# avabag01-ai/spectrogram-midi

Measured on AMD Instinct MI355X. Metric: audio-seconds transcribed/sec (44.1 kHz, n_fft=2048), higher is better.
Workload: dtype f64

## Files before the change

spectrogram-midi_amd/csrc/kernels.hip:

```cpp
#include "kernels.h"
#include "fft8.h"
#include "rake_decide.h"

#include <algorithm>
#include <cfloat>
#include <cmath>
#include <cstdlib>
#include <cstring>
#include <type_traits>

namespace aegis {

__device__ __forceinline__ int find_clip(const int64_t *__restrict__ frame_off, int n_clips, int64_t f) {
    int lo = 0, hi = n_clips;
    while (hi - lo > 1) {
        const int mid = (lo + hi) >> 1;
        if (frame_off[mid] <= f) lo = mid; else hi = mid;
    }
    return lo;
}

__device__ __forceinline__ int64_t geo_n_sel(const PassParams &p) { return p.ctl ? p.ctl->n_sel : p.n_sel; }
__device__ __forceinline__ int64_t geo_t_begin(const PassParams &p) { return p.ctl ? p.ctl->t_begin : p.t_begin; }
__device__ __forceinline__ int64_t geo_vt_begin(const PassParams &p) { return p.ctl ? p.ctl->vt_begin : p.vt_begin; }
// ... 343 lines not shown
                    v[q] = make_double2((double)xs[i], i < 1024 ? (double)xs[1024 - i] : 0.0);
                }
                fft8_pass1_write(z, tid, v);
                __syncthreads();
                if (want_rms && tid < 16) {
                    const float *r = red + tid * 8;
                    blk[tid] = ((r[0] + r[1]) + (r[2] + r[3])) + ((r[4] + r[5]) + (r[6] + r[7]));
                }
                fft8_read8(z, tid, v);
                __syncthreads();
                fft8_pass_write<8>(z, tid, v, twr.p2);
                __syncthreads();
                fft8_read8(z, tid, v);
                __syncthreads();
                fft8_pass_write<64>(z, tid, v, twr.p3);
                __syncthreads();
                fft8_pass4(z, tid, twr);
                __syncthreads();
            }
            FRM_TICK(2)
            if (want_rms && tid == 0 && live) {
                float b0 = (blk[0] + blk[1]) + (blk[2] + blk[3]);
                float b1 = (blk[4] + blk[5]) + (blk[6] + blk[7]);
                float b2 = (blk[8] + blk[9]) + (blk[10] + blk[11]);
                float b3 = (blk[12] + blk[13]) + (blk[14] + blk[15]);
                const float total = 0.0f + ((b0 + b1) + (b2 + b3));
                p.out_rms[fo] = sqrtf(total / 2048.0f);
            }
            if (!want_fft) continue;

            if (tid < 205) {
                auto zpair = [&](int k, double2 &zk, double2 &zn) { zk = z[zsw(k & 2047)]; zn = z[zsw((2048 - k) & 2047)]; };
                auto Afrom = [](const double2 &zk, const double2 &zn) { return make_double2(zk.x + zn.x, zk.y - zn.y); };
                const int k0 = 5 * tid;
                double2 zk, zn, zk1, zn1;
                zpair(k0 - 1, zk, zn);
                double2 Am = Afrom(zk, zn);
                zpair(k0, zk, zn);
                double2 A = Afrom(zk, zn);
#pragma unroll
                for (int r = 0; r < 5; ++r) {
                    const int k = k0 + r;
                    zpair(k + 1, zk1, zn1);
                    const double2 Ap = Afrom(zk1, zn1);
                    if (want_pyin) {
                        const double2 Bv = make_double2(zk.y + zn.y, zn.x - zk.x);
                        P[h][r] = c_mul(A, Bv);
                    }
                    if (want_mel) {
                        const float re = (float)(0.125 * (2.0 * A.x - (Am.x + Ap.x)));
                        const float im = (float)(0.125 * (2.0 * A.y - (Am.y + Ap.y)));
                        const float mag = (float)sqrt((double)re * (double)re + (double)im * (double)im);
                        (h == 0 ? pw : pw1)[k] = mag * mag;
                    }
                    Am = A; A = Ap; zk = zk1; zn = zn1;
                }
            }
            if (want_mel && h == 1 && tid < 15) pw1[1025 + tid] = 0.0f;
            __syncthreads();
            FRM_TICK(3)
        }
        __builtin_amdgcn_s_waitcnt(kWaitVmcnt0);
        if (want_mel) {
            if (has_chunk) {
                const float4 *wp = reinterpret_cast<const float4 *>(tb.mel_chunk_w) + tid * 4;
                const float4 w0 = wp[0], w1 = wp[1], w2 = wp[2], w3 = wp[3];
#pragma unroll
                for (int h = 0; h < 2; ++h) {
                    const float *pp = (h == 0 ? pw : pw1) + mel_bin;
                    float acc = 0.0f;
                    acc = fmaf(w0.x, pp[0], acc); acc = fmaf(w0.y, pp[1], acc); acc = fmaf(w0.z, pp[2], acc); acc = fmaf(w0.w, pp[3], acc);
                    acc = fmaf(w1.x, pp[4], acc); acc = fmaf(w1.y, pp[5], acc); acc = fmaf(w1.z, pp[6], acc); acc = fmaf(w1.w, pp[7], acc);
                    acc = fmaf(w2.x, pp[8], acc); acc = fmaf(w2.y, pp[9], acc); acc = fmaf(w2.z, pp[10], acc); acc = fmaf(w2.w, pp[11], acc);
                    acc = fmaf(w3.x, pp[12], acc); acc = fmaf(w3.y, pp[13], acc); acc = fmaf(w3.z, pp[14], acc); acc = fmaf(w3.w, pp[15], acc);
                    (h == 0 ? part : part1)[tid] = acc;
                }
            }
            __syncthreads();
            {
                const int h = wid >> 1, bt = tid & 127;
                const bool live = flive[h];
                const float *pt = h == 0 ? part : part1;
                float acc = 0.0f;
                if (bt < p.n_mels && live) {
                    const int c0 = band_c0, c1 = band_c1;
                    float pv[6];
#pragma unroll
                    for (int k = 0; k < 6; ++k) pv[k] = pt[min(c0 + k, 255)];
                    acc = c0 < c1 ? pv[0] : 0.0f;
#pragma unroll
                    for (int k = 1; k < 6; ++k) if (c0 + k < c1) acc = acc + pv[k];
                    for (int cidx = c0 + 6; cidx < c1; ++cidx) acc = acc + pt[cidx];
                    p.melpow[fidx[h] * p.n_mels + bt] = acc;
                }
                const unsigned m = wave_umax(__float_as_uint(acc));
                if (lane == 0 && live) atomicMax(&p.clipmax[fclip[h]], m);
            }
            if (!want_pyin) __syncthreads();
        }
        FRM_TICK(4)
        if (!want_pyin) continue;

        if (tid < 205) {
#pragma unroll
            for (int r = 0; r < 5; ++r) {
                const int k = 5 * tid + r;
                const double2 u = P[0][r], v = P[1][r];
                z[zsw(k)] = make_double2(u.x - v.y, -u.y - v.x);
                if (k > 0 && k < 1024) z[zsw(2048 - k)] = make_double2(u.x + v.y, u.y - v.x);
            }
        }
        __syncthreads();
        {
            double2 v[8];
            fft8_read8(z, tid, v);
            __syncthreads();
            fft8_pass1_write(z, tid, v);
            __syncthreads();
            fft8_read8(z, tid, v);
            __syncthreads();
            fft8_pass_write<8>(z, tid, v, twr.p2);
            __syncthreads();
            fft8_read8(z, tid, v);
            __syncthreads();
            fft8_pass_write<64>(z, tid, v, twr.p3);
            __syncthreads();
            fft8_pass4_lags(z, tid, twr, mp);
            __syncthreads();
        }
        FRM_TICK(5)
        const bool keep_first = p.cmnd_in_frame != 0;
        if (keep_first) {
            float es[2][3];
#pragma unroll
            for (int h = 0; h < 2; ++h) {
                const float *row = en + (pr + h) * en_stride;
                float en0 = row[0];
                if (fabsf(en0) < 1e-6f) en0 = 0.0f;
#pragma unroll
                for (int u = 0; u < 3; ++u) {
                    float e = row[min(tid + 256 * u, mp)];
                    if (fabsf(e) < 1e-6f) e = 0.0f;
                    es[h][u] = en0 + e;
                }
            }
            __syncthreads();
            double *__restrict__ d0 = reinterpret_cast<double *>(en + pr * en_stride);
            double *__restrict__ d1 = p.dfn + fidx[1] * (int64_t)p.lag_stride;
#pragma unroll
            for (int u = 0; u < 3; ++u) {
                const int tau = tid + 256 * u;
                if (tau <= mp) {
                    const double2 zz = z[zsw(1024 + tau)];
                    double a0 = zz.x * (1.0 / 8192.0), a1 = -zz.y * (1.0 / 8192.0);
                    if (fabs(a0) < 1e-6) a0 = 0.0;
                    if (fabs(a1) < 1e-6) a1 = 0.0;
                    if constexpr (INJECT) {
                        if (flive[0]) d0[tau] = inj[fout[0] * (int64_t)(mp + 1) + tau];
                        if (flive[1]) d1[tau] = inj[fout[1] * (int64_t)(mp + 1) + tau];
                    } else {
                        if (flive[0]) d0[tau] = (double)es[0][u] - 2.0 * a0;
                        if (flive[1]) d1[tau] = (double)es[1][u] - 2.0 * a1;
                    }
                }
            }
        } else {
#pragma unroll
        for (int h = 0; h < 2; ++h) {
            if (!flive[h]) continue;
            const float *row = en + (pr + h) * en_stride;
            float en0 = row[0];
            if (fabsf(en0) < 1e-6f) en0 = 0.0f;
            double *__restrict__ drow = p.dfn + fidx[h] * (int64_t)p.lag_stride;
            for (int tau = tid; tau <= mp; tau += 256) {
                const double2 zz = z[zsw(1024 + tau)];
                double a = (h == 0 ? zz.x : -zz.y) * (1.0 / 8192.0);
                if (fabs(a) < 1e-6) a = 0.0;
                float e = row[tau];
                if (fabsf(e) < 1e-6f) e = 0.0f;
                const float esum = en0 + e;
                if constexpr (INJECT) drow[tau] = inj[fout[h] * (int64_t)(mp + 1) + tau];
                else drow[tau] = (double)esum - 2.0 * a;
            }
        }
        }
        FRM_TICK(6)
    }
    if (want_pyin && p.cmnd_in_frame) {
        const int RS = frame_cmnd_stride(mp), minp = p.min_period;
        double *zrows = reinterpret_cast<double *>(fsm);
        auto row_of = [&](int i) { return (i & 1) ? zrows + (i >> 1) * RS : reinterpret_cast<double *>(en + i * en_stride); };
        __syncthreads();
        double dv[kFramesPerWg][3];
        int64_t fr[kFramesPerWg];
#pragma unroll
        for (int i = 0; i < kFramesPerWg; ++i) fr[i] = i < nfr ? frow[i] : -1;
#pragma unroll
        for (int i = 0; i < kFramesPerWg; ++i) {
            const double *__restrict__ src = (i & 1) ? p.dfn + (fr[i] < 0 ? 0 : fr[i]) * (int64_t)p.lag_stride : row_of(i);
#pragma unroll
            for (int u = 0; u < 3; ++u) {
                const int tau = tid + 256 * u;
                dv[i][u] = (fr[i] >= 0 && tau <= mp) ? src[tau] : 0.0;
            }
        }
#pragma unroll
        for (int i = 1; i < kFramesPerWg; i += 2) {
#pragma unroll
            for (int u = 0; u < 3; ++u) {
                const int tau = tid + 256 * u;
                if (i < nfr && tau <= mp) zrows[(i >> 1) * RS + tau] = dv[i][u];
            }
        }
        __syncthreads();
        FRM_TICK(7)
        if (wid == 0) __builtin_amdgcn_s_setprio(3);
        if (wid == 0 && lane < nfr) cmnd_walk(row_of(lane), mp);
        if (wid == 0) __builtin_amdgcn_s_setprio(0);
        __syncthreads();
        FRM_TICK(8)
        const bool troughs = p.troughs != 0;
#pragma unroll
        for (int i = 0; i < kFramesPerWg; ++i) {
            double *__restrict__ drow = p.dfn + (fr[i] < 0 ? 0 : fr[i]) * (int64_t)p.lag_stride;
            double *__restrict__ cs = row_of(i);
#pragma unroll
            for (int u = 0; u < 3; ++u) {
                const int tau = tid + 256 * u;
                if (fr[i] >= 0 && tau >= minp && tau <= mp) {
                    const double yv = dv[i][u] / (cs[tau] / (double)tau + DBL_MIN);
                    if (troughs) cs[tau] = yv;
                    else drow[tau] = yv;
                }
            }
        }
        FRM_TICK(9)
        if (troughs) {
            __syncthreads();
            const int nl = p.n_lags, KM = trough_km(nl), NR = (nl + 63) >> 6;
            const unsigned long long below = (1ull << lane) - 1ull;
            for (int i = wid; i < nfr; i += 4) {
                if (fr[i] < 0) continue;
                const double *__restrict__ y = row_of(i) + minp;
                double *__restrict__ trow = p.dfn + fr[i] * (int64_t)p.lag_stride;
                int16_t *__restrict__ tiv = reinterpret_cast<int16_t *>(trow + 8 + 2 * KM);
                int K = 0;
                for (int r = 0; r < NR; ++r) {
                    const int k = 64 * r + lane;
                    bool tr = false;
                    double ym = 0.0, y0 = 0.0, yp = 0.0;
                    if (k < nl) {
                        y0 = y[k];
                        if (k > 0) ym = y[k - 1];
                        if (k < nl - 1) yp = y[k + 1];
                        if (k == 0) tr = y0 < yp;
                        else if (k == nl - 1) tr = y0 < ym;
                        else tr = (y0 < ym) && (y0 <= yp);
                    }
                    const unsigned long long m = __ballot(tr);
                    if (tr) {
                        const int pos = K + __popcll(m & below);
                        double shift = 0.0;
                        if (k > 0 && k < nl - 1) {
                            const double a = yp + ym - 2.0 * y0;
                            const double b = (yp - ym) / 2.0;
                            if (fabs(b) < fabs(a)) shift = -b / a;
                        }
                        trow[8 + pos] = y0;
                        trow[8 + KM + pos] = shift;
                        tiv[pos] = (int16_t)k;
                    }
                    K += __popcll(m);
                }
                if (lane == 0) trow[0] = __longlong_as_double((long long)K);
            }
        }
    }
#if defined(AEGIS_ABLATE) && (AEGIS_ABLATE & 128)
    if (blockIdx.x == 1000 && (tid == 0 || tid == 64)) { for (int k = 0; k < 10; ++k) g_frm_dbg[(tid ? 12 : 0) + k] = facc[k]; }
#endif
}
#if defined(AEGIS_ABLATE) && (AEGIS_ABLATE & 128)
hipError_t frame_debug_fetch(long long *dst) { return hipMemcpyFromSymbol(dst, HIP_SYMBOL(g_frm_dbg), sizeof(long long) * 24); }
#else
hipError_t frame_debug_fetch(long long *dst) { for (int i = 0; i < 24; ++i) dst[i] = 0; return hipSuccess; }
#endif

constexpr int kKMax = 512;
constexpr int kMaxRounds = 8;

template <int CTRL, int ROW_MASK>
__device__ __forceinline__ int dpp_imin(int v) {
    return min(v, __builtin_amdgcn_update_dpp(v, v, CTRL, ROW_MASK, 0xf, false));
}
__device__ __forceinline__ int wave_min_i32(int v) {
    v = dpp_imin<0x111, 0xf>(v);
    v = dpp_imin<0x112, 0xf>(v);
    v = dpp_imin<0x114, 0xf>(v);
    v = dpp_imin<0x118, 0xf>(v);
    v = dpp_imin<0x142, 0xa>(v);
    v = dpp_imin<0x143, 0xc>(v);
    return __builtin_amdgcn_readlane(v, 63);
}

__device__ __forceinline__ void wave_sync() {
    __builtin_amdgcn_fence(__ATOMIC_SEQ_CST, "wavefront");
    __builtin_amdgcn_wave_barrier();
}

#if defined(AEGIS_ABLATE) && (AEGIS_ABLATE & 256)
__device__ long long g_obs_dbg[16];
#define OBS_TICK(k) { const long long now__ = clock64(); oacc[k] += now__ - olast; olast = now__; }
#else
#define OBS_TICK(k)
#endif
__global__ __launch_bounds__(512, 4) void pyin_obs_kernel(PassParams p, DevTables tb, int frames_per_wave) {
    extern __shared__ __align__(16) unsigned char osm[];
    const int nl = p.n_lags, B = p.n_bins;
    const int KM = nl / 2 + 2;
    const int YN = (max(nl, B) + 1) & ~1;
    const int DN = (p.max_period + 1 + 32 + 1) & ~1;
    const int UN = (max(DN, 2 * KM + (4 * KM + 7) / 8) + 1) & ~1;
    const int TN = (2 * (KM + 1) + 101 + 1) & ~1;
    const int lane = threadIdx.x & 63;
    const int wid = __builtin_amdgcn_readfirstlane((int)(threadIdx.x >> 6)), nwaves = (int)(blockDim.x >> 6);
    double *bfact = reinterpret_cast<double *>(osm);
    double *bexp = bfact + (KM + 1);
    double *bcum = bexp + (KM + 1);
    double *y = bfact + TN + (size_t)wid * (YN + UN);
    double *row = y;
    double *dd = y + YN;
    double *th = dd;
    double *tp = th + KM;
    int16_t *ti = reinterpret_cast<int16_t *>(tp + KM);
    int16_t *tbin = ti + KM;
    __shared__ double beta_s[104];

#if defined(AEGIS_ABLATE) && (AEGIS_ABLATE & 256)
    long long oacc[12] = {0, 0, 0, 0, 0, 0, 0, 0, 0, 0, 0, 0}, olast = clock64();
#endif
    for (int i = threadIdx.x; i < 100; i += blockDim.x) beta_s[i] = tb.beta_probs[i];
    for (int i = threadIdx.x; i <= KM; i += blockDim.x) { bfact[i] = tb.boltz_fact[i]; bexp[i] = tb.boltz_exp[i]; }
    for (int i = threadIdx.x; i <= 100; i += blockDim.x) bcum[i] = tb.beta_cumsum[i];
    __syncthreads();

    int64_t f = 0, fo = 0, sel_end = 0;
    int Kn = -1;
    const int64_t n_sel = geo_n_sel(p);
    for (int it = 0; it < frames_per_wave; ++it) {
    const int64_t fsel = ((int64_t)blockIdx.x * nwaves + wid) * frames_per_wave + it;
    if (fsel >= n_sel) break;
    if (it > 0 && fsel < sel_end) { ++f; ++fo; }
    else {
        int c;
        int64_t t;
        map_frame(p, fsel, c, t, f);
        fo = out_index(p, c, t);
        sel_end = p.sel_off[c + 1];
    }
    const int mp = p.max_period, minp = p.min_period;
    const double *__restrict__ dr = p.dfn + f * (int64_t)p.lag_stride;
    wave_sync();
    int K = 0;
    double *tsh = y;
    if (p.troughs) {
        const int KMt = trough_km(nl);
        if (Kn >= 0) K = Kn;
        else {
        K = __builtin_amdgcn_readfirstlane((int)__double_as_longlong(dr[0]));
        const int16_t *__restrict__ tiv = reinterpret_cast<const int16_t *>(dr + 8 + 2 * KMt);
        for (int k = lane; k < K; k += 64) {
            const double h = dr[8 + k], sh = dr[8 + KMt + k];
            const int16_t ix = tiv[k];
            th[k] = h; tsh[k] = sh; ti[k] = ix;
        }
        }
        wave_sync();
        OBS_TICK(0)
    } else {
    if (p.cmnd_in_frame) {
        for (int base = lane; base < nl; base += 320) {
            double t5[5];
#pragma unroll
            for (int u = 0; u < 5; ++u) t5[u] = dr[minp + min(base + 64 * u, nl - 1)];
#pragma unroll
            for (int u = 0; u < 5; ++u) if (base + 64 * u < nl) y[base + 64 * u] = t5[u];
        }
        wave_sync();
        OBS_TICK(0)
    } else {
    for (int base = lane; base <= mp; base += 320) {
        double t5[5];
#pragma unroll
        for (int u = 0; u < 5; ++u) t5[u] = dr[min(base + 64 * u, mp)];
#pragma unroll
        for (int u = 0; u < 5; ++u) if (base + 64 * u <= mp) dd[base + 64 * u] = t5[u];
    }
    wave_sync();
    OBS_TICK(0)
    if (lane == 0) {
        double cs = dd[1];
        if (minp <= 1) y[1 - minp] = cs;
        int tau = 2;
        constexpr int GL = 8;
        double2 ra[GL / 2], rb[GL / 2];
        auto request = [&](double2 (&r)[GL / 2], int t0) {
#pragma unroll
            for (int i = 0; i < GL / 2; ++i) r[i] = *reinterpret_cast<const double2 *>(dd + t0 + 2 * i);
        };
        auto group = [&](auto all_tag, double2 (&cur)[GL / 2], double2 (&nxt)[GL / 2], int t0) {
            constexpr bool ALL = decltype(all_tag)::value;
            request(nxt, t0 + GL);
            double *yo = y + (t0 - minp);
#pragma unroll
            for (int i = 0; i < GL / 2; ++i) {
                cs = cs + cur[i].x; if (ALL || t0 + 2 * i >= minp) yo[2 * i] = cs;
                cs = cs + cur[i].y; if (ALL || t0 + 2 * i + 1 >= minp) yo[2 * i + 1] = cs;
            }
        };
        request(ra, tau);
        bool in_a = true;
        for (; tau < minp && tau + GL - 1 <= mp; tau += GL, in_a = !in_a) {
            if (in_a) group(std::false_type{}, ra, rb, tau); else group(std::false_type{}, rb, ra, tau);
        }
        if (!in_a && tau + GL - 1 <= mp) { group(std::true_type{}, rb, ra, tau); tau += GL; }
        for (; tau + 2 * GL - 1 <= mp; tau += 2 * GL) { group(std::true_type{}, ra, rb, tau); group(std::true_type{}, rb, ra, tau + GL); }
        if (tau + GL - 1 <= mp) { group(std::true_type{}, ra, rb, tau); tau += GL; }
        for (; tau <= mp; ++tau) { cs = cs + dd[tau]; if (tau >= minp) y[tau - minp] = cs; }
    }
    wave_sync();
    OBS_TICK(1)
    for (int i = lane; i < nl; i += 64) {
        const int tau = i + minp;
        y[i] = dd[tau] / (y[i] / (double)tau + DBL_MIN);
    }
    if (p.yin != nullptr) {
        wave_sync();
        double *__restrict__ yo = p.yin + f * (int64_t)p.yin_stride;
        for (int i = lane; i < nl; i += 64) yo[i] = y[i];
    }
    wave_sync();
    }

    OBS_TICK(2)
    const int CH = (nl + 63) >> 6;
    unsigned mask = 0;
    int cnt = 0;
    for (int r = 0; r < CH; ++r) {
        const int i = lane * CH + r;
        if (i < nl) {
            const double yi = y[i];
            bool tr;
            if (i == 0) tr = yi < y[1];
            else if (i == nl - 1) tr = yi < y[i - 1];
            else tr = (yi < y[i - 1]) && (yi <= y[i + 1]);
            if (tr) { mask |= 1u << r; ++cnt; }
        }
    }
    const int incl = wave_incl_scan(cnt, lane);
    K = __shfl(incl, 63);
    {
        int k = incl - cnt;
        for (int r = 0; r < CH; ++r)
            if (mask & (1u << r)) { const int i = lane * CH + r; th[k] = y[i]; ti[k] = (int16_t)i; ++k; }
    }
    wave_sync();
    }

    OBS_TICK(3)
    double vp = 0.0;
    unsigned segm = 0;
    const int rounds = (K + 63) >> 6;
    const bool ahead = p.troughs && it + 1 < frames_per_wave && fsel + 1 < sel_end;
    double nK = 0.0, nh[2] = {0.0, 0.0}, nsh[2] = {0.0, 0.0};
    int16_t nix[2] = {0, 0};
    auto tail = [&](auto maxr_tag) {
        constexpr int MAXR = decltype(maxr_tag)::value;
        if (K > 0) {
            int jk[MAXR];
            double acc[MAXR];
            int jmin = 101;
    #pragma unroll
            for (int q = 0; q < MAXR; ++q) {
                jk[q] = 101; acc[q] = 0.0;
                if (q < rounds) {
                    const int k = q * 64 + lane;
                    if (k < K) {
                        const double h = th[k];
                        int g;
                        if (!(h < 1.0)) g = 100;
                        else if (h <= 0.0) g = 0;
                        else g = (int)(h * 100.0);
                        auto thr = [](int i) { return i >= 100 ? 1.0 : (double)i * 0.01; };
                        while (g < 100 && !(h < thr(g + 1))) ++g;
                        while (g > 0 && h < thr(g)) --g;
                        jk[q] = g;
                        jmin = min(jmin, g);
                    }
                }
            }
            jmin = wave_min_i32(jmin);
            OBS_TICK(4)

            const unsigned long long lt_mask = (1ull << lane) - 1ull;
            int j = jmin;
            while (j < 100) {
                unsigned long long M[MAXR];
                int nj = 0, nxt = 100;
    #pragma unroll
                for (int q = 0; q < MAXR; ++q) {
                    M[q] = 0ull;
                    if (q < rounds) {
                        M[q] = __ballot(jk[q] <= j);
                        nj += __popcll(M[q]);
                        if (jk[q] > j) nxt = min(nxt, jk[q]);
                    }
                }
                nxt = wave_min_i32(nxt);
                const double fact = bfact[nj];
                double prior[MAXR];
                int before = 0;
    #pragma unroll
                for (int q = 0; q < MAXR; ++q) {
                    prior[q] = 0.0;
                    if (q < rounds) {
                        if (jk[q] <= j) prior[q] = fact * bexp[before + __popcll(M[q] & lt_mask)];
                        before += __popcll(M[q]);
                    }
                }
                for (int jj = j; jj < nxt; ++jj) {
                    const double bj = beta_s[jj];
    #pragma unroll
                    for (int q = 0; q < MAXR; ++q)
                        if (q < rounds) acc[q] = acc[q] + prior[q] * bj;
                }
                j = nxt;
            }

            OBS_TICK(5)
            double bh = INFINITY;
            int bk = kKMax;
    #pragma unroll
            for (int q = 0; q < MAXR; ++q) {
                const int k = q * 64 + lane;
                if (q < rounds && k < K) { const double h = th[k]; if (h < bh) { bh = h; bk = k; } }
            }
    #pragma unroll
            for (int o = 32; o >= 1; o >>= 1) {
                const double oh = __shfl_xor(bh, o);
                const int ok = __shfl_xor(bk, o);
                if (oh < bh || (oh == bh && ok < bk)) { bh = oh; bk = ok; }
            }
    #pragma unroll
            for (int q = 0; q < MAXR; ++q) {
                if (q < rounds && q * 64 + lane == bk) {
                    const int nb = jk[q] > 100 ? 100 : jk[q];
                    acc[q] = acc[q] + 0.01 * bcum[nb];
                }
            }

    #pragma unroll
            for (int q = 0; q < MAXR; ++q) {
                const int k = q * 64 + lane;
                if (q < rounds && k < K) {
                    const double pr = acc[q];
                    int bin = -1;
                    if (pr != 0.0) {
                        const int i = ti[k];
                        double shift = 0.0;
                        if (p.troughs) shift = tsh[k];
                        else if (i > 0 && i < nl - 1) {
                            const double ym = y[i - 1], y0 = y[i], yp = y[i + 1];
                            const double a = yp + ym - 2.0 * y0;
                            const double b = (yp - ym) / 2.0;
                            if (fabs(b) < fabs(a)) shift = -b / a;
                        }
                        const double period = (double)(p.min_period + i) + shift;
                        const double f0c = (double)p.sr / period;
                        double r = rint(120.0 * log2(f0c / p.fmin));
                        r = !(r >= 0.0) ? 0.0 : (r > (double)B ? (double)B : r);
                        bin = (int)r;
                    }
                    tp[k] = pr;
                    tbin[k] = (int16_t)bin;
                }
            }
        }
        OBS_TICK(6)
        if (ahead) {
            const int KMt = trough_km(nl);
            const double *__restrict__ drn = dr + p.lag_stride;
            const int16_t *__restrict__ tivn = reinterpret_cast<const int16_t *>(drn + 8 + 2 * KMt);
            nK = drn[0];
    #pragma unroll
            for (int q = 0; q < 2; ++q) {
                const int k = min(q * 64 + lane, KMt - 1);
                nh[q] = drn[8 + k]; nsh[q] = drn[8 + KMt + k]; nix[q] = tivn[k];
            }
        }
        wave_sync();
        for (int b = lane; b < B; b += 64) row[b] = p.log_tiny;
        wave_sync();
        if (K > 0) {
            bool winq[MAXR];
            double prq[MAXR];
            unsigned lseg = 0;
            int binq[MAXR];
            unsigned long long hasm[MAXR];
    #pragma unroll
            for (int q = 0; q < MAXR; ++q) {
                const int k = q * 64 + lane;
                binq[q] = (q < rounds && k < K) ? (int)tbin[k] : -1;
                hasm[q] = __ballot(binq[q] >= 0);
            }
    #pragma unroll
            for (int q = 0; q < MAXR; ++q) {
                winq[q] = false; prq[q] = 0.0;
                const int bin = binq[q];
                if (bin >= 0 && bin < B) {
                    const unsigned long long above = lane < 63 ? hasm[q] >> (lane + 1) : 0ull;
                    int k2 = -1;
                    if (above) k2 = q * 64 + lane + (int)__ffsll((long long)above);
                    else {
    #pragma unroll
                        for (int q2 = MAXR - 1; q2 > q; --q2)
                            if (hasm[q2]) k2 = q2 * 64 + (int)__ffsll((long long)hasm[q2]) - 1;
                    }
                    const bool win = (k2 < 0) || ((int)tbin[k2 < 0 ? 0 : k2] != bin);
                    if (win) { prq[q] = tp[q * 64 + lane]; row[bin] = log(prq[q] + DBL_MIN); lseg |= 1u << (bin >> 6); }
                    winq[q] = win;
                }
            }
            double s = 0.0;
    #pragma unroll
            for (int q = MAXR - 1; q >= 0; --q) {
                if (q < rounds) {
                    unsigned long long m = __ballot(winq[q]);
                    while (m) {
                        const int l = 63 - __clzll((long long)m);
                        const double v = __hiloint2double(__builtin_amdgcn_readlane(__double2hiint(prq[q]), l),
                                                          __builtin_amdgcn_readlane(__double2loint(prq[q]), l));
                        s = s + v;
                        m &= ~(1ull << l);
                    }
                }
            }
            vp = s < 0.0 ? 0.0 : (s > 1.0 ? 1.0 : s);
            for (int sg = 0; sg * 64 < B; ++sg)
                if (__ballot((lseg >> sg) & 1u)) segm |= 1u << sg;
        }
    };
    if (rounds <= 2) tail(std::integral_constant<int, 2>{});
    else tail(std::integral_constant<int, kMaxRounds>{});
    wave_sync();
    OBS_TICK(7)
    Kn = -1;
    if (ahead) {
        __builtin_amdgcn_s_waitcnt(kWaitVmcnt0);
        Kn = __builtin_amdgcn_readfirstlane((int)__double_as_longlong(nK));
        if (Kn > 128) Kn = -1;
    #pragma unroll
        for (int q = 0; q < 2; ++q) {
            const int k = q * 64 + lane;
            if (k < Kn) { th[k] = nh[q]; ti[k] = nix[q]; }
        }
    }
    const double unv = (1.0 - vp) / (double)B;
    if (unv == 0.0) segm = 0x40000000u | ((1u << ((B + 63) >> 6)) - 1u);
    double *__restrict__ orow = p.logobs + f * (int64_t)p.obs_stride;
    for (int b = lane, sg = 0; b < B; b += 64, ++sg)
        if ((segm >> sg) & 1u) orow[b] = row[b];
    if (lane == 0) {
        p.obs_seg[f] = (int32_t)segm;
        p.logunv[f] = log(unv + DBL_MIN);
        if (p.out_vprob != nullptr) p.out_vprob[fo] = vp;
    }
    #pragma unroll
    for (int q = 0; q < 2; ++q) {
        const int k = q * 64 + lane;
        if (k < Kn) y[k] = nsh[q];
    }
    OBS_TICK(8)
    }
#if defined(AEGIS_ABLATE) && (AEGIS_ABLATE & 256)
    if (blockIdx.x == 100 && threadIdx.x == 0) { for (int k = 0; k < 9; ++k) g_obs_dbg[k] = oacc[k]; g_obs_dbg[9] = frames_per_wave; }
#endif
}
#if defined(AEGIS_ABLATE) && (AEGIS_ABLATE & 256)
hipError_t obs_debug_fetch(long long *dst) { return hipMemcpyFromSymbol(dst, HIP_SYMBOL(g_obs_dbg), sizeof(long long) * 16); }
#else
hipError_t obs_debug_fetch(long long *dst) { for (int i = 0; i < 16; ++i) dst[i] = 0; return hipSuccess; }
#endif

__global__ __launch_bounds__(256) void decode_kernel(PassParams p, DevTables tb) {
    const int64_t f = (int64_t)blockIdx.x * 256 + threadIdx.x;
    if (f >= p.n_frames) return;
    const int s = p.states[f];
    const bool voiced = (unsigned)s < (unsigned)p.n_bins;
    const int c = find_clip(p.frame_off, p.n_clips, f);
    const int64_t fo = out_index(p, c, f - p.frame_off[c]);
    if (p.out_voiced != nullptr) p.out_voiced[fo] = voiced ? 1 : 0;
    if (p.out_f0 != nullptr) p.out_f0[fo] = voiced ? tb.freqs[s] : p.f0_unvoiced;
    if (p.out_bin != nullptr) p.out_bin[fo] = voiced ? (int16_t)s : (int16_t)-1;
}

__global__ __launch_bounds__(256) void db_rake_kernel(PassParams p) {
    __shared__ float tile[64][129];
    __shared__ int rclip[64];
    const int tid = threadIdx.x, lane = tid & 63, wid = tid >> 6;
    const int nm = p.n_mels;
    const int64_t fb = (int64_t)blockIdx.x * 64;
    for (int rr = 0; rr < 16; ++rr) {
        const int r = wid * 16 + rr;
        const int64_t f = fb + r;
        if (f >= p.n_frames) { if (lane == 0) rclip[r] = -1; continue; }
        const int c = find_clip(p.frame_off, p.n_clips, f);
        if (lane == 0) rclip[r] = c;
        const float ref = fmaxf(1e-10f, __uint_as_float(p.clipmax[c]));
        const float refdb = 10.0f * (float)log10((double)ref);
        float cmax = -INFINITY;
        for (int m = lane; m < nm; m += 64) {
            const float s = fmaxf(1e-10f, p.melpow[f * nm + m]);
            float v = 10.0f * (float)log10((double)s);
            v = v - refdb;
            v = fmaxf(v, 0.0f - 80.0f);
            tile[r][m] = v;
            cmax = fmaxf(cmax, v);
        }
#pragma unroll
        for (int o = 32; o >= 1; o >>= 1) cmax = fmaxf(cmax, __shfl_xor(cmax, o));
        int active = 0;
        const float thr = cmax - 20.0f;
        for (int m0 = 0; m0 < nm; m0 += 64) {
            const int m = m0 + lane;
            const bool on = (m < nm) && (tile[r][m] > thr);
            active += __popcll(__ballot(on));
        }
        if (lane == 0) {
            bool cand = false;
            if (!(cmax < -60.0f)) cand = ((double)active / (double)nm) > p.rake_ratio;
            p.rake_raw[f] = cand ? 1 : 0;
        }
    }
    __syncthreads();
    if (p.out_colmean != nullptr && tid < 64 && rclip[tid] >= 0) {
        const int c = rclip[tid], mid = nm / 2;
        const float *row = tile[tid];
        float a = row[0];
        for (int m = 1; m < mid; ++m) a = a + row[m];
        const float lo_sum = a;
        float hs = row[mid];
        for (int m = mid + 1; m < nm; ++m) hs = hs + row[m];
        for (int m = max(mid, 1); m < nm; ++m) a = a + row[m];
        const int64_t fo = out_index(p, c, fb + tid - p.frame_off[c]);
        p.out_colmean[fo] = a / (float)nm;
        p.out_colmean[p.out_total + fo] = mid > 0 ? lo_sum / (float)mid : NAN;
        p.out_colmean[2 * p.out_total + fo] = hs / (float)(nm - mid);
    }
    if (p.out_sdb != nullptr) {
        for (int idx = tid; idx < 64 * nm; idx += 256) {
            const int m = idx >> 6, r = idx & 63;
            const int c = rclip[r];
            if (c < 0) continue;
            const int64_t fo = p.frame_off[c];
            const int64_t Fc = p.frame_off[c + 1] - fo;
            const int64_t tl = fb + r - fo;
            p.out_sdb[(int64_t)nm * p.out_off[c] + (int64_t)m * Fc + tl] = tile[r][m];
        }
    }
}

constexpr int kRakeRows = 5;
struct RakeLane { float smax; int sure, ntop, n; };
__device__ __forceinline__ void rake_rows_load(float (&a)[kRakeRows], float (&b)[kRakeRows], const float *__restrict__ base,
                                               int r0, int nrows, int nm, int lane) {
#pragma unroll
    for (int i = 0; i < kRakeRows; ++i) {
        const float *row = base + (int64_t)min(r0 + i, nrows - 1) * nm;
        a[i] = row[min(lane, nm - 1)];
        b[i] = row[min(lane + 64, nm - 1)];
    }
}
__device__ __forceinline__ void rake_rows_classify(const float (&a)[kRakeRows], const float (&b)[kRakeRows], int r0, int nrows, int nm,
                                                   int lane, float (*lst)[64], RakeLane &mine) {
    const bool va = lane < nm, vb = lane + 64 < nm;
#pragma unroll
    for (int i = 0; i < kRakeRows; ++i) {
        const int r = r0 + i;
        if (r >= nrows) break;
        const float sa = rake_floor(a[i]), sb = rake_floor(b[i]);
        const float smax = __uint_as_float(wave_umax(max(va ? __float_as_uint(sa) : 0u, vb ? __float_as_uint(sb) : 0u)));
        const RakeWindow w = rake_window(smax);
        const unsigned long long sure_a = __ballot(va && rake_sure_active(sa, w)), sure_b = __ballot(vb && rake_sure_active(sb, w));
        const unsigned long long top_a = __ballot(va && rake_top_listed(sa, w)), top_b = __ballot(vb && rake_top_listed(sb, w));
        const unsigned long long mid_a = __ballot(va && rake_mid_listed(sa, w)), mid_b = __ballot(vb && rake_mid_listed(sb, w));
        const int sure = __popcll(sure_a) + __popcll(sure_b);
        const int ntop_a = __popcll(top_a), ntop = ntop_a + __popcll(top_b);
        const int nmid_a = __popcll(mid_a), n = ntop + nmid_a + __popcll(mid_b);
        const bool walk = !w.usable || n > kRakeListCap;
        if (n != 0 && !walk) {
            const unsigned long long below = (1ull << lane) - 1ull;
            if ((top_a >> lane) & 1ull) lst[__popcll(top_a & below)][r] = sa;
            if ((top_b >> lane) & 1ull) lst[ntop_a + __popcll(top_b & below)][r] = sb;
            if ((mid_a >> lane) & 1ull) lst[ntop + __popcll(mid_a & below)][r] = sa;
            if ((mid_b >> lane) & 1ull) lst[ntop + nmid_a + __popcll(mid_b & below)][r] = sb;
        }
        if (lane == r) { mine.smax = smax; mine.sure = sure; mine.ntop = ntop; mine.n = walk ? -1 : n; }
    }
}
__global__ __launch_bounds__(256) void rake_pow_kernel(PassParams p) {
    __shared__ float lst[4][kRakeListCap][64];
    const int lane = threadIdx.x & 63, wid = __builtin_amdgcn_readfirstlane((int)(threadIdx.x >> 6));
    const int nm = p.n_mels;
    const int64_t f0 = ((int64_t)blockIdx.x * 4 + wid) * 64;
    if (f0 >= p.n_frames) return;
    const int nrows = (int)min((int64_t)64, p.n_frames - f0);
    const float *__restrict__ base = p.melpow + f0 * nm;
    float a0[kRakeRows], b0[kRakeRows], a1[kRakeRows], b1[kRakeRows];
    rake_rows_load(a0, b0, base, 0, nrows, nm, lane);
    const int64_t f = f0 + min(lane, nrows - 1);
    const int c_first = find_clip(p.frame_off, p.n_clips, f0), c_last = find_clip(p.frame_off, p.n_clips, f0 + nrows - 1);
    const int c = c_first == c_last ? c_first : find_clip(p.frame_off, p.n_clips, f);
    const float refdb = rake_refdb(rake_floor(__uint_as_float(p.clipmax[c])));
    RakeLane mine = {0.0f, 0, 0, 0};
    for (int r0 = 0; r0 < nrows; r0 += 2 * kRakeRows) {
        rake_rows_load(a1, b1, base, r0 + kRakeRows, nrows, nm, lane);
        rake_rows_classify(a0, b0, r0, nrows, nm, lane, lst[wid], mine);
        rake_rows_load(a0, b0, base, r0 + 2 * kRakeRows, nrows, nm, lane);
        rake_rows_classify(a1, b1, r0 + kRakeRows, nrows, nm, lane, lst[wid], mine);
    }
    if (lane >= nrows) return;
    int active;
    if (mine.n < 0) active = rake_column_full(base + (int64_t)lane * nm, nm, refdb);
    else active = rake_decide(mine.smax, mine.sure, mine.ntop, mine.n, &lst[wid][0][lane], 64, refdb);
    p.rake_raw[f] = rake_candidate(active, nm, p.rake_ratio) ? 1 : 0;
}

__global__ __launch_bounds__(256) void rake_runs_kernel(PassParams p) {
    const int64_t f = (int64_t)blockIdx.x * 256 + threadIdx.x;
// ... 221 lines not shown
```

Measured before the change: 307,800.

## Precompute threshold-change set via wave OR bitmask and broadcast beta via readlane

Replaces the per-iteration wave-min search for the next threshold index with a one-time wave-wide OR of a 100-bit occupancy mask, then walks set bits with ctz. Beta values are held in registers across lanes and broadcast with readlane instead of being read from LDS in the inner accumulation loop. For the two-round case the next change step's ballot and table lookups are issued before the accumulation stretch to overlap latency. This trades repeated cross-lane reductions and LDS loads for extra registers and more complex control flow.

Result: faster. 312,700, median of 6 (+1.6%).

```diff
diff --git a/spectrogram-midi_amd/csrc/kernels.hip b/spectrogram-midi_amd/csrc/kernels.hip
--- a/spectrogram-midi_amd/csrc/kernels.hip
+++ b/spectrogram-midi_amd/csrc/kernels.hip
@@ -669,6 +669,19 @@
     v = dpp_imin<0x143, 0xc>(v);
     return __builtin_amdgcn_readlane(v, 63);
 }
+template <int CTRL, int ROW_MASK>
+__device__ __forceinline__ unsigned dpp_or(unsigned v) {
+    return v | (unsigned)__builtin_amdgcn_update_dpp((int)v, (int)v, CTRL, ROW_MASK, 0xf, false);
+}
+__device__ __forceinline__ unsigned wave_or_u32(unsigned v) {
+    v = dpp_or<0x111, 0xf>(v);
+    v = dpp_or<0x112, 0xf>(v);
+    v = dpp_or<0x114, 0xf>(v);
+    v = dpp_or<0x118, 0xf>(v);
+    v = dpp_or<0x142, 0xa>(v);
+    v = dpp_or<0x143, 0xc>(v);
+    return (unsigned)__builtin_amdgcn_readlane((int)v, 63);
+}
 
 __device__ __forceinline__ void wave_sync() {
     __builtin_amdgcn_fence(__ATOMIC_SEQ_CST, "wavefront");
@@ -846,7 +859,7 @@
         if (K > 0) {
             int jk[MAXR];
             double acc[MAXR];
-            int jmin = 101;
+            const double blo = beta_s[lane], bhi = beta_s[min(64 + lane, 99)];
     #pragma unroll
             for (int q = 0; q < MAXR; ++q) {
                 jk[q] = 101; acc[q] = 0.0;
@@ -862,46 +875,73 @@
                         while (g < 100 && !(h < thr(g + 1))) ++g;
                         while (g > 0 && h < thr(g)) --g;
                         jk[q] = g;
-                        jmin = min(jmin, g);
                     }
                 }
             }
-            jmin = wave_min_i32(jmin);
             OBS_TICK(4)
 
-            const unsigned long long lt_mask = (1ull << lane) - 1ull;
-            int j = jmin;
+            constexpr bool AHEAD = MAXR == 2;
+            const int blo_l = __double2loint(blo), blo_h = __double2hiint(blo), bhi_l = __double2loint(bhi), bhi_h = __double2hiint(bhi);
+            unsigned long long left_lo, left_hi;
+            {
+                unsigned w[4] = {0u, 0u, 0u, 0u};
+    #pragma unroll
+                for (int q = 0; q < MAXR; ++q) {
+                    const unsigned bit = jk[q] < 100 ? 1u << (jk[q] & 31) : 0u;
+    #pragma unroll
+                    for (int i = 0; i < 4; ++i) w[i] |= (jk[q] >> 5) == i ? bit : 0u;
+                }
+    #pragma unroll
+                for (int i = 0; i < 4; ++i) w[i] = wave_or_u32(w[i]);
+                left_lo = ((unsigned long long)w[1] << 32) | w[0];
+                left_hi = ((unsigned long long)w[3] << 32) | w[2];
+            }
+            auto take_next = [&]() {
+                const bool in_lo = left_lo != 0ull;
+                const unsigned long long m = in_lo ? left_lo : left_hi, rest = m & (m - 1ull);
+                const int r = m ? (in_lo ? 0 : 64) + (int)__builtin_ctzll(m) : 100;
+                left_lo = in_lo ? rest : 0ull;
+                left_hi = in_lo ? left_hi : rest;
+                return r;
+            };
+            auto change = [&](int j0, int &nxt, double &fact, double (&e)[MAXR]) {
+                unsigned long long M[MAXR];
+                int nj = 0;
+    #pragma unroll
+                for (int q = 0; q < MAXR; ++q) {
+                    M[q] = __ballot(jk[q] <= j0);
+                    nj += __popcll(M[q]);
+                }
+                fact = bfact[nj];
+                int before = 0;
+    #pragma unroll
+                for (int q = 0; q < MAXR; ++q) {
+                    e[q] = bexp[before + (int)__builtin_amdgcn_mbcnt_hi((unsigned)(M[q] >> 32), __builtin_amdgcn_mbcnt_lo((unsigned)M[q], 0u))];
+                    before += __popcll(M[q]);
+                }
+                nxt = take_next();
+            };
+            auto stretch = [&](const double (&prior)[MAXR], int lo_l, int lo_h, int jj, int jend, int off) {
+                for (; jj < jend; ++jj) {
+                    const double bj = __hiloint2double(__builtin_amdgcn_readlane(lo_h, jj - off), __builtin_amdgcn_readlane(lo_l, jj - off));
+    #pragma unroll
+                    for (int q = 0; q < MAXR; ++q)
+                        if (MAXR == 2 || q < rounds) acc[q] = acc[q] + prior[q] * bj;
+                }
+            };
+            int j = take_next(), nxt = 100;
+            double fact = 0.0, e[MAXR];
+            change(j, nxt, fact, e);
             while (j < 100) {
-                unsigned long long M[MAXR];
-                int nj = 0, nxt = 100;
-    #pragma unroll
-                for (int q = 0; q < MAXR; ++q) {
-                    M[q] = 0ull;
-                    if (q < rounds) {
-                        M[q] = __ballot(jk[q] <= j);
-                        nj += __popcll(M[q]);
-                        if (jk[q] > j) nxt = min(nxt, jk[q]);
-                    }
-                }
-                nxt = wave_min_i32(nxt);
-                const double fact = bfact[nj];
                 double prior[MAXR];
-                int before = 0;
-    #pragma unroll
-                for (int q = 0; q < MAXR; ++q) {
-                    prior[q] = 0.0;
-                    if (q < rounds) {
-                        if (jk[q] <= j) prior[q] = fact * bexp[before + __popcll(M[q] & lt_mask)];
-                        before += __popcll(M[q]);
-                    }
-                }
-                for (int jj = j; jj < nxt; ++jj) {
-                    const double bj = beta_s[jj];
-    #pragma unroll
-                    for (int q = 0; q < MAXR; ++q)
-                        if (q < rounds) acc[q] = acc[q] + prior[q] * bj;
-                }
-                j = nxt;
+    #pragma unroll
+                for (int q = 0; q < MAXR; ++q) prior[q] = jk[q] <= j ? fact * e[q] : 0.0;
+                const int j1 = nxt;
+                if (AHEAD) change(j1, nxt, fact, e);
+                stretch(prior, blo_l, blo_h, j, min(j1, 64), 0);
+                stretch(prior, bhi_l, bhi_h, max(j, 64), j1, 64);
+                if (!AHEAD) change(j1, nxt, fact, e);
+                j = j1;
             }
 
             OBS_TICK(5)
```
